# xiph/daala

Measured on AMD Instinct MI355X. Metric: 1080p all-intra transform blocks/s (filter+DCT+PVQ), higher is better.
Workload: dtype int32 (lifting DCT/filters) + f64 (PVQ search)

## Files before the change

### daala_amd/api.py

```python
import ctypes
import os

import numpy as np

_HERE = os.path.dirname(os.path.abspath(__file__))
_LIB = None


class DaalaHipError(RuntimeError):
    pass


EXPERIMENTS_LIB = os.path.join(_HERE, "lib", "libdaalahip_exp.so")


def lib_path():
    return os.environ.get("ODHIP_LIB") or os.path.join(_HERE, "lib", "libdaalahip.so")


def lib():
    global _LIB
    if _LIB is None:
        path = lib_path()
        if not os.path.exists(path):
# ... 515 lines not shown
REFBAND_R_NULL, REFBAND_THETA, REFBAND_NOREF, REFBAND_FLIP, REFBAND_UNCERTAIN = 1, 2, 4, 8, 16
REFITEM_SEARCHED, REFITEM_WITH_REF, REFITEM_K_RANGE = 1, 2, 4
REFITEM_MOMENT_SHIFT = 8


class _RefJob(ctypes.Structure):
    _fields_ = [("d_coef", ctypes.c_void_p), ("d_ref", ctypes.c_void_p), ("nplanes", ctypes.c_int),
                ("w", ctypes.c_int), ("h", ctypes.c_int), ("bs", ctypes.c_int),
                ("is_keyframe", ctypes.c_int), ("pli", ctypes.c_int), ("d_qm", ctypes.c_void_p),
                ("d_qm_inv", ctypes.c_void_p), ("q_band", ctypes.POINTER(ctypes.c_int32)),
                ("beta_band", ctypes.POINTER(ctypes.c_int32)), ("band", ctypes.c_void_p),
                ("items", ctypes.c_void_p), ("y", ctypes.c_void_p), ("r16", ctypes.c_void_p),
                ("x16", ctypes.c_void_p), ("xr", ctypes.c_void_p), ("d_rate", ctypes.c_void_p),
                ("choice", ctypes.c_void_p), ("d_dq", ctypes.c_void_p),
                ("q_band2", ctypes.POINTER(ctypes.c_int32)), ("plane_split", ctypes.c_int),
                ("luma", ctypes.c_void_p), ("d_q_plane", ctypes.c_void_p)]


class PvqRefJob:

    def __init__(self, coef, ref, bs, qm, qm_inv, q_band, beta_band, is_keyframe, pli, rate=None,
                 share=None, q_band2=None, plane_split=0):
        import torch
        _need(coef, torch.int32, "coef")
        _need(ref, torch.int32, "ref")
        assert coef.shape == ref.shape
        self.coef, self.ref, self.bs, self.qm, self.qm_inv = coef, ref, int(bs), qm, qm_inv
        self.is_keyframe, self.pli, self.rate = int(is_keyframe), int(pli), rate
        nplanes, h, w = coef.shape
        n = 4 << bs
        self.nblocks = B = nplanes * (h // n) * (w // n)
# ... 292 lines not shown


PIPE_STAGES = ("image_copy_pad_luma", "forward_pyramid_luma", "pvq_noref_bands", "pvq_choose",
               "cfl_refs_from_luma", "dequant_inverse_luma", "image_copy_pad_chroma",
               "forward_pyramid_chroma", "pvq_ref_bands", "pvq_ref_choose", "dequant_inverse_chroma")
(BUF_PIC, BUF_PX, BUF_LEVEL, BUF_RECON, BUF_BAND, BUF_Y, BUF_CHOICE, BUF_ITEMS, BUF_REF,
 BUF_RATE) = range(10)
BUF_PRED = 10


class _PipeConfig(ctypes.Structure):
    _fields_ = [("device", ctypes.c_int), ("frames", ctypes.c_int), ("pic_w", ctypes.c_int),
                ("pic_h", ctypes.c_int), ("chroma_cfl", ctypes.c_int), ("serial", ctypes.c_int),
                ("price", ctypes.c_int), ("fpr_bits", ctypes.c_int), ("inter", ctypes.c_int),
                ("chroma_444", ctypes.c_int),
                ("pvq_norm_lambda", ctypes.c_double), ("quant", ctypes.c_void_p)]


def export_layout_make(nblocks, bs, with_ref):
    lay = _ExportLayout()
    n = len(bs)
    _check(lib().odhip_export_layout_make(ctypes.byref(lay), n, (ctypes.c_long * n)(*nblocks), (ctypes.c_int * n)(*bs),
                                          (ctypes.c_int * n)(*[int(bool(w)) for w in with_ref])),
           "odhip_export_layout_make")
    return lay, _layout_dict(lay)


def _layout_dict(lay):
    secs = [{k: int(getattr(lay.section[i], k)) for k in ("bs", "ngroups", "cap_words", "blocks_per_group", "record_bytes",
                                                         "nrecords", "records_off", "group_base_off", "stream_off")}
            for i in range(lay.nsections)]
# ... 55 lines not shown
class _ExportSection(ctypes.Structure):
    _fields_ = [("bs", ctypes.c_int32), ("ngroups", ctypes.c_uint32), ("cap_words", ctypes.c_uint32),
                ("blocks_per_group", ctypes.c_uint32), ("record_bytes", ctypes.c_uint32), ("pad", ctypes.c_uint32),
                ("nrecords", ctypes.c_uint64), ("records_off", ctypes.c_uint64),
                ("group_base_off", ctypes.c_uint64), ("stream_off", ctypes.c_uint64)]


class _ExportLayout(ctypes.Structure):
    _fields_ = [("nsections", ctypes.c_int32), ("pad", ctypes.c_int32), ("fixed_bytes", ctypes.c_uint64),
                ("total_bytes", ctypes.c_uint64), ("section", _ExportSection * 16)]


class Pipe:

    def __init__(self, quant, frames, pic_w, pic_h, chroma_cfl=True, serial=False, device=0,
                 pvq_norm_lambda=0.147, price=False, fpr_bits=0, inter=False, chroma_444=False):
        L = lib()
        L.odhip_pipe_create.restype = ctypes.c_void_p
        L.odhip_pipe_theta_reruns.restype = ctypes.c_long
        L.odhip_pipe_price_reruns.restype = ctypes.c_long
        cfg = _PipeConfig(int(device), int(frames), int(pic_w), int(pic_h), int(bool(chroma_cfl)),
                          int(bool(serial)), int(bool(price)), int(fpr_bits), int(bool(inter)),
                          int(bool(chroma_444)),
                          float(pvq_norm_lambda),
                          ctypes.cast(ctypes.byref(quant.c), ctypes.c_void_p))
        self.h = L.odhip_pipe_create(ctypes.byref(cfg))
        if not self.h:
            raise DaalaHipError("odhip_pipe_create failed")
        self.frames, self.pic_w, self.pic_h = int(frames), int(pic_w), int(pic_h)
        self.W, self.H = (pic_w + 63) & ~63, (pic_h + 63) & ~63
        self.chroma_cfl = bool(chroma_cfl)
        self.fpr_bits = int(fpr_bits)
        self.inter = bool(inter)
        self.chroma_444 = bool(chroma_444)
        cdec = 0 if chroma_444 else 1
        self.cw, self.ch = (self.pic_w + cdec) >> cdec, (self.pic_h + cdec) >> cdec
        self.chroma_levels = int(L.odhip_pipe_chroma_levels(self._p()))
        global _pipes
        if _pipes is None:
            import weakref
# ... 561 lines not shown
```

### daala_amd/csrc/lapped_kernels.hip

```cpp
#include "../../include/daala_hip.h"
#include <stdio.h>
#include <stdlib.h>
#include <string.h>
#include <type_traits>
#include "od_ctx.cuh"
#include "od_tile.cuh"
#include "od_pvq_math.cuh"
#include "gen/od_scan_tables.h"

namespace {

__device__ __forceinline__ void od_lds_barrier() {
  asm volatile("s_waitcnt lgkmcnt(0)\n\ts_barrier" ::: "memory");
}

typedef int od_v4i __attribute__((ext_vector_type(4)));
__device__ __forceinline__ void od_store_coef4(od_coeff *p, int4 v) {
#ifdef OD_PYR_STORE_NT
  od_v4i w = {v.x, v.y, v.z, v.w};
  __builtin_nontemporal_store(w, reinterpret_cast<od_v4i *>(p));
#else
  *reinterpret_cast<int4 *>(p) = v;
#endif
}
// ... 595 lines not shown
  int pic_w;
  int pic_h;
  int leaf_bs;
  const int16_t *y;
  const int4 *choice;
  const int16_t *qm_inv;
  long nblocks;
  int len;
  int nb_bands;
  const int16_t *r16;
  const od_coeff *ref;
  int px16;
  int inter;
  int dbg;
  int wide;
};

constexpr int kMaxInvLevels = 5;
struct InverseArgsMulti {
  InverseArgs a[kMaxInvLevels];
  int nplanes;
};

__device__ __attribute__((aligned(16))) unsigned short gInvScanXY[OD_SCAN_LEN];
__device__ unsigned char gInvBandOf[OD_SCAN_LEN];

__device__ __forceinline__ unsigned char od_to_px(int c) {
  return (unsigned char)min(max(((c + 8) >> 4) + 128, 0), 255);
}
__device__ __forceinline__ short od_to_px16(int c) {
  return (short)min(max(c + 2048, 0), 4095);
}
__device__ __forceinline__ void od_store_px(uint8_t *plane, long at, int c, bool px16) {
  if (px16) reinterpret_cast<short *>(plane)[at] = od_to_px16(c);
  else plane[at] = od_to_px(c);
}

struct OdQ16 {
  int sh;
  int sl;
  __device__ __forceinline__ explicit OdQ16(int scale) : sh(scale >> 16), sl(scale & 0xffff) {}
  __device__ __forceinline__ int mul(int y) const { return __mul24(y, sh) + (__mul24(y, sl) >> 16); }
};
__device__ __forceinline__ int od_pulse16(unsigned w, int odd) {
  return odd ? (int)w >> 16 : (int)(w << 16) >> 16;
}

template <int LEAF>
__device__ __forceinline__ int walk_band_of(int j, int &off) {
  int b = 0;
  off = 1;
  if constexpr (LEAF >= 1) {
    if (j >= 16) { b = 1; off = 16; }
    if (j >= 24) { b = 2; off = 24; }
    if (j >= 32) { b = 3; off = 32; }
  }
  if constexpr (LEAF >= 2) {
    if (j >= 64) { b = 4; off = 64; }
    if (j >= 96) { b = 5; off = 96; }
    if (j >= 128) { b = 6; off = 128; }
// ... 391 lines not shown
        const int4 ch = chs[hf];
        const int rnd = (1 << ch.w) >> 1;
        const OdQ16 sc(ch.z);
#pragma unroll
        for (int e = 0; e < 4; e++) {
#pragma unroll
          for (int u = 0; u < 2; u++) {
            const int yv = od_pulse16((unsigned)yd[e], u);
            const int qmi = u ? qd[e] >> 16 : (int)(short)qd[e];
            const int xy = u ? (unsigned)sd[e] >> 16 : sd[e] & 0xffff;
            int v = (__mul24(sc.mul(yv), qmi) + rnd) >> ch.w;
            if (hf == 0 && e == 0 && u == 0 && j0 == 0) v = dc;
            t[base + (xy >> 8)*P + (xy & 255)] = v;
          }
        }
      }
    }
  }
  else {
    load_plane_tile<TILE>(t, a.coef + plane_off, a.w, x0, y0, tid);
  }
  __syncthreads();
  switch (a.leaf_bs) {
    case 0: if constexpr (MINLEAF <= 0 && MAXLEAF >= 0) inverse_leaf<TILE, 0>(t, tid); break;
    case 1: if constexpr (MINLEAF <= 1 && MAXLEAF >= 1) inverse_leaf<TILE, 1>(t, tid); break;
    case 2: if constexpr (MINLEAF <= 2 && MAXLEAF >= 2) inverse_leaf<TILE, 2>(t, tid); break;
    case 3: if constexpr (MINLEAF <= 3 && MAXLEAF >= 3) inverse_leaf<TILE, 3>(t, tid); break;
    default:
      if constexpr (TILE == 64 && MAXLEAF >= 4) inverse_leaf<TILE, 4>(t, tid);
      break;
// ... 73 lines not shown
#pragma unroll
      for (int e = 0; e < 4; e++) {
#pragma unroll
        for (int u = 0; u < 2; u++) {
          const int yv = od_pulse16((unsigned)yd[e], u);
          const int qmi = u ? qd[e] >> 16 : (int)(short)qd[e];
          const int xy = u ? (unsigned)sd[e] >> 16 : sd[e] & 0xffff;
          int v = (__mul24(sc.mul(yv), qmi) + rnd) >> ch.w;
          if (hf == 0 && e == 0 && u == 0 && j0 == 0) v = dc;
          tt[base + (xy >> 8)*P + (xy & 255)] = v;
        }
      }
    }
  }
  __syncthreads();
  if (a.leaf_bs == 3) {
    const int s2 = tid >> 7;
    const int lt = tid & 127;
    od_tile_rows<TILE, 3, true, T, 128>(t[s2], t[s2], lt, OdAllBlocks());
    __syncthreads();
    od_tile_cols<TILE, 3, true, T, 128>(t[s2], t[s2], lt, OdAllBlocks());
    __syncthreads();
  }
  else {
    const int g = tid >> 6;
    if (tid < 64) {
      int *tt = t[tid >> 5];
      const int base = (tid & 31)*P;
      T in[64];
      T out[64];
// ... 730 lines not shown
    if constexpr (SRC == 1) {
      if (!OD_INV_DBG(a, 4)) {
        if (!ahead) {
          f.heads(a, plane, plane_off, xg, y0, tid);
          f.pulses(a, plane, xg, y0, tid);
        }
        if constexpr (Fetch::len < Fetch::n*Fetch::n) {
          walk_zero<TILE, G, NT>(t, tid);
          od_lds_barrier();
        }
        if (leaf4) f.commit_leaf4(t, a, tid);
        else f.commit(t, a, tid);
      }
      else walk_zero<TILE, G, NT>(t, tid);
      od_lds_barrier();
      if (ahead && g + 1 < g1) f.heads(a, plane, plane_off, xg + G*TILE, y0, tid);
    }
    else if (leaf4) {
      if constexpr (LEAF == 0 && SRC == 2) walk_leaf4<TILE, G, NT, SRC>(t, a, plane, plane_off, xg, y0, tid);
      od_lds_barrier();
    }
    else {
      if (OD_INV_DBG(a, 4)) walk_zero<TILE, G, NT>(t, tid);
      else if constexpr (SRC == 0) walk_load_plane<TILE, G, NT>(t, a.coef + plane_off, a.w, xg, y0, tid);
      else if constexpr (SRC == 2) walk_load_ref<TILE, G, NT, LEAF>(t, a, plane, plane_off, xg, y0, tid);
      od_lds_barrier();
    }
    if (!leaf4 && !OD_INV_DBG(a, 16)) {
      walk_idct_pass<TILE, G, NT, LEAF, true>(t, tid);
      od_lds_barrier();
// ... 553 lines not shown
  return inverse_launch(ia, nlevels, nplanes, dec, (hipStream_t)stream);
}

extern "C" int odhip_inverse_level_pvq(uint8_t *d_px, int px_stride, long px_plane_stride,
 const odhip_pvq_job *job, int dec, int pic_w, int pic_h, odhip_stream stream) {
  InverseArgs ia;
  int rc = pvq_inverse_args(ia, d_px, px_stride, px_plane_stride, job, dec, pic_w, pic_h);
  if (rc) return rc;
  rc = upload_inv_tables();
  if (rc) return rc;
  return inverse_launch(ia, job->nplanes, dec, (hipStream_t)stream);
}

extern "C" int odhip_inverse_levels_pvq(uint8_t *const *d_px, int px_stride, long px_plane_stride,
 const odhip_pvq_job *jobs, int njobs, int dec, int pic_w, int pic_h, odhip_stream stream) {
  if (!d_px || !jobs || njobs <= 0 || njobs > kMaxInvLevels) return ODHIP_EINVAL;
  InverseArgs ia[kMaxInvLevels];
  for (int i = 0; i < njobs; i++) {
    const int rc = pvq_inverse_args(ia[i], d_px[i], px_stride, px_plane_stride, &jobs[i], dec, pic_w,
     pic_h);
    if (rc) return rc;
    if (jobs[i].nplanes != jobs[0].nplanes || jobs[i].w != jobs[0].w || jobs[i].h != jobs[0].h) {
      return ODHIP_EINVAL;
    }
  }
  const int rc = upload_inv_tables();
  if (rc) return rc;
  return inverse_launch(ia, njobs, jobs[0].nplanes, dec, (hipStream_t)stream);
}

extern "C" int odhip_inverse_levels_pvq_ref(uint8_t *const *d_px, int px_stride, long px_plane_stride,
 const odhip_pvq_refjob *jobs, int njobs, int dec, int pic_w, int pic_h, odhip_stream stream) {
  if (!d_px || !jobs || njobs <= 0 || njobs > kMaxInvLevels || (dec != 0 && dec != 1)) return ODHIP_EINVAL;
  InverseArgs ia[kMaxInvLevels];
  for (int i = 0; i < njobs; i++) {
    const odhip_pvq_refjob &j = jobs[i];
    const bool lref = j.luma != nullptr && j.is_keyframe && j.pli != 0;
    if ((!j.d_ref && !lref) || !j.r16 || ((uintptr_t)j.r16 & 15) || j.nplanes != jobs[0].nplanes || j.w != jobs[0].w
// ... 16 lines not shown
```

### daala_amd/csrc/pipeline.hip

```cpp
#include <stdio.h>
#include <stdlib.h>
#include <string.h>
#include <atomic>
#include <chrono>
#include <vector>
#include "od_ctx.cuh"
#include "gen/od_scan_tables.h"

namespace {

constexpr int kStages = ODHIP_PIPE_NSTAGES;
constexpr int kMaxTimed = 4096;

struct PlaneSet {
  int dec;
  int pli;
  int nplanes;
  int w, h;
  int pw, ph;
  int nlev;
  uint8_t *pic;
  uint8_t *pic_buf[2];
  uint8_t *px;
  uint8_t *pred_pic;
// ... 52 lines not shown

struct odhip_pipe {
  odhip_pipe_config cfg = {};
  int pic_w = 0, pic_h = 0, W = 0, H = 0;
  odhip_ctx *ctx[2] = {};
  hipStream_t stream[2] = {};
  bool serial = false;
  PlaneSet set[2] = {};
  int cdec = 1;
  odhip_pvq_job jobs[2][2*ODHIP_NBSIZES] = {};
  int njobs = 0;
  odhip_pvq_refjob refjobs[2][ODHIP_NBSIZES] = {};
  odhip_pvq_refjob interjobs[2][ODHIP_NBSIZES] = {};
  bool inter_pending[2] = {};
  double *rate[2][ODHIP_NBSIZES] = {};
  hipEvent_t ev_refs[2] = {};
  hipEvent_t ev_used[2] = {};
  long nstep = 0;
  int pending = -1;
  long reruns = 0;
  long price_reruns = 0;
  double wait_ms = 0;
  long k_range = 0;
  bool record = false;
  hipStream_t copy_stream = nullptr;
  hipEvent_t ev_fed = nullptr;
  hipEvent_t ev_pad[2] = {};
  int front = 0;
  bool fed = false;
  hipStream_t export_stream = nullptr;
// ... 225 lines not shown
  }
  p->njobs = 0;
  return ODHIP_SUCCESS;
}

int setup_keyframe_jobs(odhip_pipe *p) {
  PlaneSet &ch = p->set[1];
  for (int bs = 0; bs < 5; bs++) STEP_TRY(setup_job(p, p->jobs[0][bs], p->set[0], bs));
  p->njobs = 5;
  if (!p->cfg.chroma_cfl) {
    for (int bs = 0; bs < ch.nlev; bs++) STEP_TRY(setup_job(p, p->jobs[0][5 + bs], ch, bs));
    p->njobs = 5 + ch.nlev;
    return ODHIP_SUCCESS;
  }
  for (int bs = 0; bs < 5; bs++) STEP_TRY(setup_job(p, p->jobs[1][bs], p->set[0], bs, &p->jobs[0][bs]));
  for (int par = 0; par < 2; par++) {
    for (int bs = 0; bs < ch.nlev; bs++) {
      STEP_TRY(setup_refjob(p, p->refjobs[par][bs], ch, bs, nullptr, par ? &p->refjobs[0][bs] : nullptr,
       &p->jobs[par][bs + ch.dec]));
    }
    STEP_TRY(pipe_event(p, &p->ev_refs[par]));
    STEP_TRY(pipe_event(p, &p->ev_used[par]));
  }
  return ODHIP_SUCCESS;
}

int pipe_init(odhip_pipe *p) {
  const odhip_pipe_config &c = p->cfg;
  ODHIP_TRY(hipSetDevice(c.device));
  p->pic_w = c.pic_w;
  p->pic_h = c.pic_h;
  p->W = (c.pic_w + 63) & ~63;
  p->H = (c.pic_h + 63) & ~63;
  p->serial = c.serial || odhip_env_serial();
// ... 190 lines not shown
}

int stage_pad_run(odhip_pipe *p, int si, hipStream_t s) {
  Timed tm(p, si ? ODHIP_PIPE_PAD_CHROMA : ODHIP_PIPE_PAD_LUMA, s);
  return pad_planes(p, si, p->set[si].px, p->set[si].pic, s);
}

int stage_pyramid(odhip_pipe *p, int si, hipStream_t s) {
  Timed tm(p, si ? ODHIP_PIPE_PYRAMID_CHROMA : ODHIP_PIPE_PYRAMID_LUMA, s);
  return pyramid(p, si, p->set[si].levels, p->set[si].px, s);
}

int stage_inverse_noref(odhip_pipe *p, int si, hipStream_t s, int jpar) {
  PlaneSet &t = p->set[si];
  Timed tm(p, si ? ODHIP_PIPE_INVERSE_CHROMA : ODHIP_PIPE_INVERSE_LUMA, s);
  return odhip_inverse_levels_pvq(t.recon, t.w, (long)t.w*t.h, p->jobs[jpar] + (si ? 5 : 0), t.nlev, t.dec,
   p->pic_w, p->pic_h, s);
}

int ref_bands(odhip_pipe *p, int si, int par, hipStream_t s) {
  const double lam = p->cfg.pvq_norm_lambda;
  const int nlev = p->set[si].nlev;
  Timed tm(p, si ? ODHIP_PIPE_BANDS_CHROMA : ODHIP_PIPE_BANDS_LUMA, s);
  if (p->cfg.price) return odhip_pvq_ref_bands_decided_multi(ref_jobs(p, si, par), nlev, lam, s);
  STEP_TRY(odhip_pvq_ref_bands_multi(ref_jobs(p, si, par), nlev, lam, s));
  return odhip_pvq_ref_resolve_begin(s);
}

int ref_choose(odhip_pipe *p, int si, int par, hipStream_t s) {
  Timed tm(p, si ? ODHIP_PIPE_CHOOSE_CHROMA : ODHIP_PIPE_CHOOSE_LUMA, s);
  return odhip_pvq_ref_choose_multi(ref_jobs(p, si, par), p->set[si].nlev, p->cfg.pvq_norm_lambda, s);
}

int ref_inverse(odhip_pipe *p, int si, int par, hipStream_t s) {
  const PlaneSet &t = p->set[si];
  Timed tm(p, si ? ODHIP_PIPE_INVERSE_CHROMA : ODHIP_PIPE_INVERSE_LUMA, s);
  return odhip_inverse_levels_pvq_ref(t.recon, t.w, (long)t.w*t.h, ref_jobs(p, si, par), t.nlev, t.dec, p->pic_w,
   p->pic_h, s);
}

// ... 297 lines not shown
  }
  return ODHIP_SUCCESS;
}

int step_cfl(odhip_pipe *p) {
  hipStream_t main = p->stream[0];
  hipStream_t side = p->stream[1];
  const int par = (int)(p->nstep & 1);
  const bool exp_on = exporting(p);
  quants_point(p, 0, par);
  {
    Current cur(p->ctx[0]);
    STEP_TRY(luma_front(p, main, par));
    STEP_TRY(luma_choose(p, main, par));
    if (exp_on) ODHIP_TRY(hipStreamWaitEvent(main, p->ev_exp_sent[par], 0));
    ODHIP_TRY(hipEventRecord(p->ev_refs[par], main));
    if (exp_on) STEP_TRY(export_luma(p, par));
    STEP_TRY(stage_inverse_noref(p, 0, main, par));
    STEP_TRY(measure(p, 0, par, main));
  }
  STEP_TRY(finish_pending(p));
  if (exp_on) STEP_TRY(export_finish(p));
  STEP_TRY(metrics_finish(p, side));
  {
    Current cur(p->ctx[1]);
    STEP_TRY(stage_pad(p, 1, side));
    STEP_TRY(stage_pyramid(p, 1, side));
    ODHIP_TRY(hipStreamWaitEvent(side, p->ev_refs[par], 0));
    quants_point(p, 1, par);
    STEP_TRY(quants_upload(p, 1, par, side));
    STEP_TRY(ref_bands(p, 1, par, side));
    ODHIP_TRY(hipEventRecord(p->ev_used[par], side));
    if (exp_on) STEP_TRY(export_chroma(p, par));
    STEP_TRY(ref_tail(p, 1, par, side));
  }
  p->pending = par;
  metrics_step_done(p, par);
  return ODHIP_SUCCESS;
}

}

extern "C" odhip_pipe *odhip_pipe_create(const odhip_pipe_config *cfg) {
  if (!cfg || !cfg->quant || cfg->frames <= 0 || cfg->pic_w <= 0 || cfg->pic_h <= 0
   || (cfg->chroma_444 != 0 && cfg->chroma_444 != 1)
   || (!cfg->chroma_444 && ((cfg->pic_w & 1) || (cfg->pic_h & 1)))
// ... 519 lines not shown
    case ODHIP_PIPE_BUF_Y:
      ptr = j ? j->cands.y : r->y;
      n = sizeof(int16_t)*(size_t)(j ? 2 : ODHIP_PVQ_REF_SLOTS)*B*len;
      break;
    case ODHIP_PIPE_BUF_CHOICE:
      ptr = j ? j->cands.choice : r->choice;
      n = sizeof(int32_t)*(size_t)B*nb*(j ? 4 : 16);
      break;
    case ODHIP_PIPE_BUF_ITEMS:
      if (!r) return ODHIP_EINVAL;
      ptr = r->items;
      n = (size_t)3*nb*ODHIP_PVQ_REF_SLOTS*B*16;
      break;
    case ODHIP_PIPE_BUF_REF:
      if (!r) return ODHIP_EINVAL;
      if (!inter) return ODHIP_EINVAL;
      ptr = t.pred_levels[level];
      n = sizeof(od_coeff)*(size_t)t.nplanes*t.w*t.h;
      break;
    case ODHIP_PIPE_BUF_RATE: {
      n = sizeof(double)*(size_t)B*nb*(j ? 2 : ODHIP_PVQ_REF_SLOTS + 1);
      if (!p->rate[set][level]) {
        ODHIP_TRY(hipSetDevice(p->cfg.device));
        PIPE_ALLOC(p, p->rate[set][level], n, true);
        for (int par = 0; par < 2; par++) {
          const JobAt a = job_at(p, set, level, par);
          if (a.ref) a.ref->d_rate = p->rate[set][level];
          else a.noref->d_rate = p->rate[set][level];
        }
      }
      ptr = p->rate[set][level];
// ... 238 lines not shown
```

### daala_amd/csrc/pvq_refbands.hip

```cpp
#include "../../include/daala_hip.h"
#include <math.h>
#include <stdio.h>
#include <stdlib.h>
#include <string.h>
#include "od_ctx.cuh"
#include "od_pvq_math.cuh"
#include "od_occupancy.cuh"
#include "od_krange.cuh"
#include "od_band_stage.cuh"
#include "gen/od_scan_tables.h"
#define OD_RSQ_TABLE_N 512
#define OD_RSQ_HUGE
#include "pvq_search.cuh"
#include "pvq_row.cuh"
#include "pvq_regs.cuh"

namespace {

constexpr int kMaxJobs = 8;
constexpr int kMaxItems = kMaxJobs*ODHIP_MAX_BANDS;
constexpr int kSlots = ODHIP_PVQ_REF_SLOTS;
constexpr int kUncCap = 1 << 16;
constexpr double kDefaultMargin = 1e-9;

// ... 27 lines not shown
  int pli;
  int q[ODHIP_MAX_BANDS];
  int beta[ODHIP_MAX_BANDS];
  int off[ODHIP_MAX_BANDS + 1];
  long split_blk;
  int q2[ODHIP_MAX_BANDS];
  const int *qp;
  unsigned plane_blocks;
  const int16_t *ly;
  const int32_t *lchoice;
  const int16_t *lqmi;
  long lnblocks;
  long lsplit;
  int llen;
  int lnb;
};

__device__ __forceinline__ int job_q(const RJob &jb, int band, long blk) {
  const int q = blk >= jb.split_blk ? jb.q2[band] : jb.q[band];
  return q ? q : jb.qp[(unsigned)blk/jb.plane_blocks*ODHIP_MAX_BANDS + band];
}

__device__ __forceinline__ void lref_piece(const RJob &jb, int band, long blk, int c0, int (&rv)[8]) {
  const long lblk = blk >= jb.lsplit ? blk - jb.lsplit : blk;
  const int4 ch = reinterpret_cast<const int4 *>(jb.lchoice)[lblk*jb.lnb + band];
  uint4 y4 = make_uint4(0, 0, 0, 0);
  if (ch.y != 0) y4 = *reinterpret_cast<const uint4 *>(jb.ly + ((long)ch.x*jb.lnblocks + lblk)*jb.llen + c0);
  const uint4 q4 = *reinterpret_cast<const uint4 *>(jb.lqmi + c0);
  const unsigned yw[4] = {y4.x, y4.y, y4.z, y4.w};
  const unsigned qw[4] = {q4.x, q4.y, q4.z, q4.w};
#pragma unroll
// ... 240 lines not shown
  const RJob &jb = it.jobs[job];
  const int band = it.band[item];
  const long blk = (long)(blockIdx.x - it.wg_start[item])*kWave + threadIdx.x;
  if (blk >= jb.nblocks) return;
  const int off = jb.off[band];
  const int w = jb.w;
  const int len = jb.len;
  const int nb_bands = jb.nb_bands;
  const int q0 = job_q(jb, band, blk);
  const int beta = jb.beta[band];
  const int is_keyframe = jb.is_keyframe;
  const int cfl_enabled = is_keyframe && jb.pli != 0;
  const long base = block_base(jb, blk);
  const od_coeff *x0 = jb.coef + base;
  const bool lref = jb.ly != nullptr;
  const od_coeff *r0 = lref ? jb.coef + base : jb.ref + base;
  const int16_t *qmp = jb.qm + off;
  odhip_pvq_refband *rec = jb.rec + blk*nb_bands;
  int16_t *x16o = jb.x16 + blk*len;
  int16_t *r16o = jb.r16 + blk*len;
  int16_t *xro = jb.xr + blk*len;
  int xv[N];
  int rv[N];
  int qm[N];
  if constexpr (N == 15) {
    int4 xr4[4];
    int4 rr4[4];
#pragma unroll
    for (int y = 0; y < 4; y++) {
      xr4[y] = *reinterpret_cast<const int4 *>(x0 + (long)y*w);
      rr4[y] = lref ? make_int4(0, 0, 0, 0) : *reinterpret_cast<const int4 *>(r0 + (long)y*w);
// ... 216 lines not shown
  const int l = lane%G;
  const long nblocks = jb.nblocks;
  const long blk0 = (long)(blockIdx.x - it.wg_start[item])*(kWave/G) + row;
  const bool live = blk0 < nblocks;
  const long blk = live ? blk0 : nblocks - 1;
  const int w = jb.w;
  const int len = jb.len;
  const int nb_bands = jb.nb_bands;
  const int q0 = job_q(jb, band, blk);
  const int beta = jb.beta[band];
  const int is_keyframe = jb.is_keyframe;
  const int cfl_enabled = is_keyframe && jb.pli != 0;
  const long base = block_base(jb, blk);
  const od_coeff *x0 = jb.coef + base;
  const bool lref = jb.ly != nullptr;
  const od_coeff *r0 = lref ? jb.coef + base : jb.ref + base;
  const int16_t *qmp = jb.qm + off + l*E;
  odhip_pvq_refband *rec = jb.rec + blk*nb_bands;
  int16_t *x16o = jb.x16 + blk*len + off;
  int16_t *r16o = jb.r16 + blk*len + off;
  int16_t *xro = jb.xr + blk*len + off;
  const int flip = cfl_enabled ? (rec[0].flags & ODHIP_REFBAND_FLIP) != 0 : 0;
  int xv[E];
  int rv[E];
  int qm[E];
  int sx = 0;
  int sr = 0;
  int nz = 0;
#pragma unroll
  for (int e = 0; e < E; e++) {
    const int pk = s_scan[l*E + e];
// ... 1653 lines not shown
    return ODHIP_EINVAL;
  }
  if (((uintptr_t)j.band & 63) || ((uintptr_t)j.items & 15) || ((uintptr_t)j.y & 15)
   || ((uintptr_t)j.r16 & 15) || ((uintptr_t)j.x16 & 15) || ((uintptr_t)j.xr & 15)
   || ((uintptr_t)j.choice & 15)) {
    return ODHIP_EINVAL;
  }
  if (mode == 0 ? (!j.d_qm || !j.x16 || !j.xr) : mode == 1 ? (!j.d_qm_inv || !j.choice || !j.d_dq)
   : !j.choice) {
    return ODHIP_EINVAL;
  }
  const int n = 4 << j.bs;
  if (j.w <= 0 || j.h <= 0 || j.w % n || j.h % n) return ODHIP_EINVAL;
  if (mode == 0 && (((uintptr_t)j.d_coef & 15) || ((uintptr_t)j.d_ref & 15))) return ODHIP_EINVAL;
  if (j.luma && !j.d_ref && mode == 1) return ODHIP_EINVAL;
  memset(&d, 0, sizeof(d));
  d.coef = j.d_coef;
  d.ref = j.d_ref;
  d.qm = j.d_qm;
  d.qm_inv = j.d_qm_inv;
  d.rec = j.band;
  d.items = j.items;
  d.y = j.y;
  d.r16 = j.r16;
  d.x16 = j.x16;
  d.xr = j.xr;
  d.rate = j.d_rate;
  d.choice = j.choice;
  d.dq = j.d_dq;
  d.nplanes = j.nplanes;
// ... 12 lines not shown
  for (int i = 0; i < d.nb_bands; i++) {
    if (j.q_band[i] < 1) return ODHIP_EINVAL;
    d.q[i] = j.q_band[i];
    d.q2[i] = j.q_band[i];
    d.beta[i] = j.beta_band[i];
  }
  d.split_blk = d.nblocks;
  if (j.q_band2) {
    if (j.plane_split <= 0 || j.plane_split >= j.nplanes) return ODHIP_EINVAL;
    d.split_blk = (long)j.plane_split*d.bw*d.bh;
    for (int i = 0; i < d.nb_bands; i++) {
      if (j.q_band2[i] < 1) return ODHIP_EINVAL;
      d.q2[i] = j.q_band2[i];
    }
  }
  d.qp = j.d_q_plane;
  d.plane_blocks = (unsigned)(d.bw*d.bh);
  if (d.qp) {
    for (int i = 0; i < d.nb_bands; i++) d.q[i] = d.q2[i] = 0;
  }
  if (j.luma) {
    const odhip_pvq_job &l = *j.luma;
    const bool up = l.bs == j.bs + 1 && l.w == 2*j.w && l.h == 2*j.h;
    const bool same = l.bs == j.bs && l.w == j.w && l.h == j.h;
    if ((!up && !same) || !l.cands.y || !l.cands.choice || !l.d_qm_inv
     || (l.nplanes != j.nplanes && 2*l.nplanes != j.nplanes) || !j.is_keyframe || j.pli == 0
     || ((uintptr_t)l.cands.y & 15) || ((uintptr_t)l.cands.choice & 15) || ((uintptr_t)l.d_qm_inv & 15)) {
      return ODHIP_EINVAL;
    }
    const int ln = 4 << l.bs;
// ... 568 lines not shown
```

### include/daala_hip.h

```cpp
#ifndef DAALA_HIP_H
#define DAALA_HIP_H
#include <stddef.h>
#include <stdint.h>

#ifdef __cplusplus
extern "C" {
#endif

typedef int32_t od_coeff;

#define ODHIP_SUCCESS (0)
#define ODHIP_EFAULT (-1)
#define ODHIP_EINVAL (-10)
#define ODHIP_EIMPL (-23)
#define ODHIP_ERANGE (-24)
#define ODHIP_EBUSY (-101)

#define ODHIP_NBSIZES 5

typedef void *odhip_stream;


typedef void (*odhip_dct_func_2d)(od_coeff *out, int out_stride,
 const od_coeff *in, int in_stride);
// ... 158 lines not shown
 double pvq_norm_lambda, odhip_stream stream);

int odhip_inverse_level_pvq(uint8_t *d_px, int px_stride, long px_plane_stride,
 const odhip_pvq_job *job, int dec, int pic_w, int pic_h, odhip_stream stream);

int odhip_cfl_refs_from_luma(const odhip_pvq_job *luma_jobs, int njobs, od_coeff *const *d_ref,
 int copies, odhip_stream stream);
int odhip_cfl_refs_from_luma_ex(const odhip_pvq_job *luma_jobs, int njobs, od_coeff *const *d_ref,
 int copies, int prezeroed, odhip_stream stream);

int odhip_pvq_profile(int enable);
int odhip_pvq_profile_read(float *ms, int max_n);

int odhip_inverse_levels_pvq(uint8_t *const *d_px, int px_stride, long px_plane_stride,
 const odhip_pvq_job *jobs, int njobs, int dec, int pic_w, int pic_h, odhip_stream stream);

int odhip_pvq_band_layout(int bs, int *nb_bands, int *offsets, int *len);

int odhip_pvq_noref_bands(const od_coeff *d_coef, int nplanes, int w, int h,
 int bs, const int16_t *d_qm, const int32_t *q_band, const int32_t *beta_band,
 double pvq_norm_lambda, const odhip_pvq_cands *out, odhip_stream stream);

int odhip_pvq_select_synth_noref(od_coeff *d_dq, const od_coeff *d_coef,
 int nplanes, int w, int h, int bs, const int16_t *d_qm_inv,
 const int32_t *q_band, const int32_t *beta_band, double pvq_norm_lambda,
 const odhip_pvq_cands *in, const double *d_rate, int32_t *d_qg_out,
 odhip_stream stream);

typedef struct {
  int32_t xshift, rshift;
// ... 76 lines not shown
  const int32_t *q_band;
  const int32_t *beta_band;
  odhip_pvq_refband *band;
  void *items;
  int16_t *y;
  int16_t *r16;
  int16_t *x16;
  int16_t *xr;
  const double *d_rate;
  int32_t *choice;
  od_coeff *d_dq;
  const int32_t *q_band2;
  int plane_split;
  const struct odhip_pvq_job_s *luma;
  const int32_t *d_q_plane;
} odhip_pvq_refjob;

int odhip_pvq_ref_set_context(int ctx);
int odhip_pvq_ref_bands_multi(const odhip_pvq_refjob *jobs, int njobs,
 double pvq_norm_lambda, odhip_stream stream);
int odhip_pvq_ref_resolve(const odhip_pvq_refjob *jobs, int njobs,
 double pvq_norm_lambda, odhip_stream stream);
int odhip_pvq_ref_resolve_begin(odhip_stream stream);
int odhip_pvq_ref_resolve_finish(const odhip_pvq_refjob *jobs, int njobs,
 double pvq_norm_lambda, odhip_stream stream);
int odhip_pvq_ref_select_synth_multi(const odhip_pvq_refjob *jobs, int njobs,
 double pvq_norm_lambda, odhip_stream stream);
int odhip_pvq_ref_profile(int enable);
int odhip_pvq_ref_profile_read(float *ms, int max_n);
int odhip_pvq_ref_choose_multi(const odhip_pvq_refjob *jobs, int njobs,
// ... 120 lines not shown

typedef struct odhip_pipe odhip_pipe;
typedef struct {
  int device;
  int frames;
  int pic_w;
  int pic_h;
  int chroma_cfl;
  int serial;
  int price;
  int fpr_bits;
  int inter;
  int chroma_444;
  double pvq_norm_lambda;
  const odhip_quant *quant;
} odhip_pipe_config;
enum {
  ODHIP_PIPE_PAD_LUMA = 0, ODHIP_PIPE_PYRAMID_LUMA, ODHIP_PIPE_BANDS_LUMA, ODHIP_PIPE_CHOOSE_LUMA,
  ODHIP_PIPE_CFL_REFS, ODHIP_PIPE_INVERSE_LUMA, ODHIP_PIPE_PAD_CHROMA, ODHIP_PIPE_PYRAMID_CHROMA,
  ODHIP_PIPE_BANDS_CHROMA, ODHIP_PIPE_CHOOSE_CHROMA, ODHIP_PIPE_INVERSE_CHROMA, ODHIP_PIPE_NSTAGES
};
enum {
  ODHIP_PIPE_BUF_PIC = 0,
  ODHIP_PIPE_BUF_PX,
  ODHIP_PIPE_BUF_LEVEL,
  ODHIP_PIPE_BUF_RECON,
  ODHIP_PIPE_BUF_BAND,
  ODHIP_PIPE_BUF_Y,
  ODHIP_PIPE_BUF_CHOICE,
  ODHIP_PIPE_BUF_ITEMS,
// ... 171 lines not shown
```

Baseline: 1.161 billion.

## Emit CfL chroma reference planes from luma inverse and share across Cb/Cr

During the luma inverse pass the kernel now writes decimated CfL reference coefficient planes straight from LDS tiles into per-level buffers. Chroma ref-band search then reads these planes directly, and Cb and Cr share one reference via a block-index offset, replacing the per-block gather from luma jobs. The chroma side stream now waits until after the luma inverse instead of after luma choose, which delays chroma start and may cost overlap. It also adds extra global stores and barriers to the inverse kernel.

New measurement: 1.125 billion. -3.1%, worse.

```diff
diff --git a/daala_amd/api.py b/daala_amd/api.py
--- a/daala_amd/api.py
+++ b/daala_amd/api.py
@@ -553,7 +553,8 @@
                 ("x16", ctypes.c_void_p), ("xr", ctypes.c_void_p), ("d_rate", ctypes.c_void_p),
                 ("choice", ctypes.c_void_p), ("d_dq", ctypes.c_void_p),
                 ("q_band2", ctypes.POINTER(ctypes.c_int32)), ("plane_split", ctypes.c_int),
-                ("luma", ctypes.c_void_p), ("d_q_plane", ctypes.c_void_p)]
+                ("luma", ctypes.c_void_p), ("d_q_plane", ctypes.c_void_p),
+                ("ref_planes", ctypes.c_int)]
 
 
 class PvqRefJob:
@@ -876,7 +877,8 @@
                 ("pic_h", ctypes.c_int), ("chroma_cfl", ctypes.c_int), ("serial", ctypes.c_int),
                 ("price", ctypes.c_int), ("fpr_bits", ctypes.c_int), ("inter", ctypes.c_int),
                 ("chroma_444", ctypes.c_int),
-                ("pvq_norm_lambda", ctypes.c_double), ("quant", ctypes.c_void_p)]
+                ("pvq_norm_lambda", ctypes.c_double), ("quant", ctypes.c_void_p),
+                ("cfl_gather", ctypes.c_int)]
 
 
 def export_layout_make(nblocks, bs, with_ref):
@@ -962,7 +964,8 @@
 class Pipe:
 
     def __init__(self, quant, frames, pic_w, pic_h, chroma_cfl=True, serial=False, device=0,
-                 pvq_norm_lambda=0.147, price=False, fpr_bits=0, inter=False, chroma_444=False):
+                 pvq_norm_lambda=0.147, price=False, fpr_bits=0, inter=False, chroma_444=False,
+                 cfl_gather=False):
         L = lib()
         L.odhip_pipe_create.restype = ctypes.c_void_p
         L.odhip_pipe_theta_reruns.restype = ctypes.c_long
@@ -971,7 +974,7 @@
                           int(bool(serial)), int(bool(price)), int(fpr_bits), int(bool(inter)),
                           int(bool(chroma_444)),
                           float(pvq_norm_lambda),
-                          ctypes.cast(ctypes.byref(quant.c), ctypes.c_void_p))
+                          ctypes.cast(ctypes.byref(quant.c), ctypes.c_void_p), int(bool(cfl_gather)))
         self.h = L.odhip_pipe_create(ctypes.byref(cfg))
         if not self.h:
             raise DaalaHipError("odhip_pipe_create failed")
diff --git a/daala_amd/csrc/lapped_kernels.hip b/daala_amd/csrc/lapped_kernels.hip
--- a/daala_amd/csrc/lapped_kernels.hip
+++ b/daala_amd/csrc/lapped_kernels.hip
@@ -633,6 +633,7 @@
   int inter;
   int dbg;
   int wide;
+  od_coeff *cfl;
 };
 
 constexpr int kMaxInvLevels = 5;
@@ -663,6 +664,28 @@
 };
 __device__ __forceinline__ int od_pulse16(unsigned w, int odd) {
   return odd ? (int)w >> 16 : (int)(w << 16) >> 16;
+}
+
+template <int G, int NT, int P>
+__device__ __forceinline__ void cfl_store(const int *t, int tile_words, const InverseArgs &a, int leaf, int plane,
+ int x0, int y0, unsigned tid) {
+  constexpr int TILE = 64;
+  constexpr int Q = G*TILE/8;
+  const int nsh = leaf + 1;
+  const unsigned nm = (1u << nsh) - 1;
+  const int cw = a.w >> 1;
+  od_coeff *out = a.cfl + ((long)plane*(a.h >> 1) + (y0 >> 1))*cw + (x0 >> 1);
+  for (unsigned i = tid; i < (unsigned)(TILE/2*Q); i += NT) {
+    const unsigned cy = i/Q;
+    const unsigned cx = (i % Q)*4;
+    const unsigned s = cx/(TILE/2);
+    const unsigned cxl = cx % (TILE/2);
+    const unsigned ly = ((cy >> nsh) << (nsh + 1)) | (cy & nm);
+    const unsigned lx = ((cxl >> nsh) << (nsh + 1)) | (cxl & nm);
+    int4 v = *reinterpret_cast<const int4 *>(t + s*tile_words + ly*P + lx);
+    if (!(cy & nm) && !(cxl & nm)) v.x = 0;
+    *reinterpret_cast<int4 *>(out + (long)cy*cw + cx) = v;
+  }
 }
 
 template <int LEAF>
@@ -1084,6 +1107,12 @@
             t[base + (xy >> 8)*P + (xy & 255)] = v;
           }
         }
+      }
+    }
+    if constexpr (TILE == 64) {
+      if (a.cfl) {
+        od_lds_barrier();
+        cfl_store<1, NT, P>(t, 0, a, a.leaf_bs, plane, x0, y0, tid);
       }
     }
   }
@@ -1187,6 +1216,10 @@
     }
   }
   __syncthreads();
+  if (a.cfl) {
+    cfl_store<2, NT, P>(&t[0][0], TILE*P, a, a.leaf_bs, plane, xb, y0, tid);
+    od_lds_barrier();
+  }
   if (a.leaf_bs == 3) {
     const int s2 = tid >> 7;
     const int lt = tid & 127;
@@ -1947,6 +1980,12 @@
       }
       else walk_zero<TILE, G, NT>(t, tid);
       od_lds_barrier();
+      if constexpr (TILE == 64 && G == 1 && LEAF >= 1) {
+        if (a.cfl) {
+          cfl_store<G, NT, P>(t, TILE*P, a, LEAF, plane, xg, y0, tid);
+          od_lds_barrier();
+        }
+      }
       if (ahead && g + 1 < g1) f.heads(a, plane, plane_off, xg + G*TILE, y0, tid);
     }
     else if (leaf4) {
@@ -2530,7 +2569,12 @@
 
 extern "C" int odhip_inverse_levels_pvq(uint8_t *const *d_px, int px_stride, long px_plane_stride,
  const odhip_pvq_job *jobs, int njobs, int dec, int pic_w, int pic_h, odhip_stream stream) {
-  if (!d_px || !jobs || njobs <= 0 || njobs > kMaxInvLevels) return ODHIP_EINVAL;
+  return odhip_inverse_levels_pvq_cfl(d_px, px_stride, px_plane_stride, jobs, njobs, dec, pic_w, pic_h, nullptr, stream);
+}
+
+extern "C" int odhip_inverse_levels_pvq_cfl(uint8_t *const *d_px, int px_stride, long px_plane_stride,
+ const odhip_pvq_job *jobs, int njobs, int dec, int pic_w, int pic_h, od_coeff *const *d_cfl, odhip_stream stream) {
+  if (!d_px || !jobs || njobs <= 0 || njobs > kMaxInvLevels || (d_cfl && dec)) return ODHIP_EINVAL;
   InverseArgs ia[kMaxInvLevels];
   for (int i = 0; i < njobs; i++) {
     const int rc = pvq_inverse_args(ia[i], d_px[i], px_stride, px_plane_stride, &jobs[i], dec, pic_w,
@@ -2538,6 +2582,10 @@
     if (rc) return rc;
     if (jobs[i].nplanes != jobs[0].nplanes || jobs[i].w != jobs[0].w || jobs[i].h != jobs[0].h) {
       return ODHIP_EINVAL;
+    }
+    if (d_cfl && d_cfl[i] && jobs[i].bs >= 1) {
+      if ((uintptr_t)d_cfl[i] & 15) return ODHIP_EINVAL;
+      ia[i].cfl = d_cfl[i];
     }
   }
   const int rc = upload_inv_tables();
diff --git a/daala_amd/csrc/pipeline.hip b/daala_amd/csrc/pipeline.hip
--- a/daala_amd/csrc/pipeline.hip
+++ b/daala_amd/csrc/pipeline.hip
@@ -90,6 +90,8 @@
   odhip_pvq_refjob interjobs[2][ODHIP_NBSIZES] = {};
   bool inter_pending[2] = {};
   double *rate[2][ODHIP_NBSIZES] = {};
+  od_coeff *cfl_plane[2][ODHIP_NBSIZES] = {};
+  bool cfl_planes = false;
   hipEvent_t ev_refs[2] = {};
   hipEvent_t ev_used[2] = {};
   long nstep = 0;
@@ -345,10 +347,15 @@
     return ODHIP_SUCCESS;
   }
   for (int bs = 0; bs < 5; bs++) STEP_TRY(setup_job(p, p->jobs[1][bs], p->set[0], bs, &p->jobs[0][bs]));
+  const char *gather = ODHIP_EXP_ENV("ODHIP_CFL_GATHER");
+  p->cfl_planes = ch.dec == 1 && !p->cfg.cfl_gather && !(gather && atoi(gather) != 0);
   for (int par = 0; par < 2; par++) {
     for (int bs = 0; bs < ch.nlev; bs++) {
       STEP_TRY(setup_refjob(p, p->refjobs[par][bs], ch, bs, nullptr, par ? &p->refjobs[0][bs] : nullptr,
        &p->jobs[par][bs + ch.dec]));
+      if (p->cfl_planes) {
+        PIPE_ALLOC(p, p->cfl_plane[par][bs], sizeof(od_coeff)*(size_t)p->set[0].nplanes*ch.w*ch.h, true);
+      }
     }
     STEP_TRY(pipe_event(p, &p->ev_refs[par]));
     STEP_TRY(pipe_event(p, &p->ev_used[par]));
@@ -569,16 +576,31 @@
 int stage_inverse_noref(odhip_pipe *p, int si, hipStream_t s, int jpar) {
   PlaneSet &t = p->set[si];
   Timed tm(p, si ? ODHIP_PIPE_INVERSE_CHROMA : ODHIP_PIPE_INVERSE_LUMA, s);
-  return odhip_inverse_levels_pvq(t.recon, t.w, (long)t.w*t.h, p->jobs[jpar] + (si ? 5 : 0), t.nlev, t.dec,
-   p->pic_w, p->pic_h, s);
-}
-
-int ref_bands(odhip_pipe *p, int si, int par, hipStream_t s) {
+  od_coeff *cfl[ODHIP_NBSIZES] = {};
+  if (si == 0 && p->cfl_planes) {
+    for (int bs = 1; bs < t.nlev; bs++) cfl[bs] = p->cfl_plane[jpar][bs - 1];
+  }
+  return odhip_inverse_levels_pvq_cfl(t.recon, t.w, (long)t.w*t.h, p->jobs[jpar] + (si ? 5 : 0), t.nlev, t.dec,
+   p->pic_w, p->pic_h, si == 0 && p->cfl_planes ? cfl : nullptr, s);
+}
+
+int ref_bands(odhip_pipe *p, int si, int par, hipStream_t s, bool planes = false) {
   const double lam = p->cfg.pvq_norm_lambda;
   const int nlev = p->set[si].nlev;
   Timed tm(p, si ? ODHIP_PIPE_BANDS_CHROMA : ODHIP_PIPE_BANDS_LUMA, s);
-  if (p->cfg.price) return odhip_pvq_ref_bands_decided_multi(ref_jobs(p, si, par), nlev, lam, s);
-  STEP_TRY(odhip_pvq_ref_bands_multi(ref_jobs(p, si, par), nlev, lam, s));
+  const odhip_pvq_refjob *jobs = ref_jobs(p, si, par);
+  odhip_pvq_refjob pj[ODHIP_NBSIZES];
+  if (planes) {
+    for (int bs = 0; bs < nlev; bs++) {
+      pj[bs] = jobs[bs];
+      pj[bs].luma = nullptr;
+      pj[bs].d_ref = p->cfl_plane[par][bs];
+      pj[bs].ref_planes = p->set[0].nplanes;
+    }
+    jobs = pj;
+  }
+  if (p->cfg.price) return odhip_pvq_ref_bands_decided_multi(jobs, nlev, lam, s);
+  STEP_TRY(odhip_pvq_ref_bands_multi(jobs, nlev, lam, s));
   return odhip_pvq_ref_resolve_begin(s);
 }
 
@@ -906,9 +928,10 @@
     STEP_TRY(luma_front(p, main, par));
     STEP_TRY(luma_choose(p, main, par));
     if (exp_on) ODHIP_TRY(hipStreamWaitEvent(main, p->ev_exp_sent[par], 0));
-    ODHIP_TRY(hipEventRecord(p->ev_refs[par], main));
+    if (!p->cfl_planes) ODHIP_TRY(hipEventRecord(p->ev_refs[par], main));
     if (exp_on) STEP_TRY(export_luma(p, par));
     STEP_TRY(stage_inverse_noref(p, 0, main, par));
+    if (p->cfl_planes) ODHIP_TRY(hipEventRecord(p->ev_refs[par], main));
     STEP_TRY(measure(p, 0, par, main));
   }
   STEP_TRY(finish_pending(p));
@@ -921,7 +944,7 @@
     ODHIP_TRY(hipStreamWaitEvent(side, p->ev_refs[par], 0));
     quants_point(p, 1, par);
     STEP_TRY(quants_upload(p, 1, par, side));
-    STEP_TRY(ref_bands(p, 1, par, side));
+    STEP_TRY(ref_bands(p, 1, par, side, p->cfl_planes));
     ODHIP_TRY(hipEventRecord(p->ev_used[par], side));
     if (exp_on) STEP_TRY(export_chroma(p, par));
     STEP_TRY(ref_tail(p, 1, par, side));
@@ -1471,7 +1494,12 @@
       break;
     case ODHIP_PIPE_BUF_REF:
       if (!r) return ODHIP_EINVAL;
-      if (!inter) return ODHIP_EINVAL;
+      if (!inter) {
+        if (set != 1 || !p->cfl_planes) return ODHIP_EINVAL;
+        ptr = p->cfl_plane[parity][level];
+        n = sizeof(od_coeff)*(size_t)p->set[0].nplanes*t.w*t.h;
+        break;
+      }
       ptr = t.pred_levels[level];
       n = sizeof(od_coeff)*(size_t)t.nplanes*t.w*t.h;
       break;
diff --git a/daala_amd/csrc/pvq_refbands.hip b/daala_amd/csrc/pvq_refbands.hip
--- a/daala_amd/csrc/pvq_refbands.hip
+++ b/daala_amd/csrc/pvq_refbands.hip
@@ -65,7 +65,13 @@
   long lsplit;
   int llen;
   int lnb;
+  long rsplit;
+  long rback;
 };
+
+__device__ __forceinline__ long ref_base(const RJob &jb, long blk, long base) {
+  return blk >= jb.rsplit ? base - jb.rback : base;
+}
 
 __device__ __forceinline__ int job_q(const RJob &jb, int band, long blk) {
   const int q = blk >= jb.split_blk ? jb.q2[band] : jb.q[band];
@@ -336,7 +342,7 @@
   const long base = block_base(jb, blk);
   const od_coeff *x0 = jb.coef + base;
   const bool lref = jb.ly != nullptr;
-  const od_coeff *r0 = lref ? jb.coef + base : jb.ref + base;
+  const od_coeff *r0 = lref ? jb.coef + base : jb.ref + ref_base(jb, blk, base);
   const int16_t *qmp = jb.qm + off;
   odhip_pvq_refband *rec = jb.rec + blk*nb_bands;
   int16_t *x16o = jb.x16 + blk*len;
@@ -583,7 +589,7 @@
   const long base = block_base(jb, blk);
   const od_coeff *x0 = jb.coef + base;
   const bool lref = jb.ly != nullptr;
-  const od_coeff *r0 = lref ? jb.coef + base : jb.ref + base;
+  const od_coeff *r0 = lref ? jb.coef + base : jb.ref + ref_base(jb, blk, base);
   const int16_t *qmp = jb.qm + off + l*E;
   odhip_pvq_refband *rec = jb.rec + blk*nb_bands;
   int16_t *x16o = jb.x16 + blk*len + off;
@@ -2267,6 +2273,8 @@
   if (j.w <= 0 || j.h <= 0 || j.w % n || j.h % n) return ODHIP_EINVAL;
   if (mode == 0 && (((uintptr_t)j.d_coef & 15) || ((uintptr_t)j.d_ref & 15))) return ODHIP_EINVAL;
   if (j.luma && !j.d_ref && mode == 1) return ODHIP_EINVAL;
+  const bool rshare = j.ref_planes != 0 && j.ref_planes != j.nplanes;
+  if (rshare && (2*j.ref_planes != j.nplanes || !j.d_ref || !j.is_keyframe || j.pli == 0 || mode == 1)) return ODHIP_EINVAL;
   memset(&d, 0, sizeof(d));
   d.coef = j.d_coef;
   d.ref = j.d_ref;
@@ -2309,6 +2317,8 @@
       d.q2[i] = j.q_band2[i];
     }
   }
+  d.rsplit = rshare ? (long)j.ref_planes*d.bw*d.bh : d.nblocks;
+  d.rback = rshare ? (long)j.ref_planes*j.w*j.h : 0;
   d.qp = j.d_q_plane;
   d.plane_blocks = (unsigned)(d.bw*d.bh);
   if (d.qp) {
diff --git a/include/daala_hip.h b/include/daala_hip.h
--- a/include/daala_hip.h
+++ b/include/daala_hip.h
@@ -196,6 +196,9 @@
 
 int odhip_inverse_levels_pvq(uint8_t *const *d_px, int px_stride, long px_plane_stride,
  const odhip_pvq_job *jobs, int njobs, int dec, int pic_w, int pic_h, odhip_stream stream);
+int odhip_inverse_levels_pvq_cfl(uint8_t *const *d_px, int px_stride, long px_plane_stride,
+ const odhip_pvq_job *jobs, int njobs, int dec, int pic_w, int pic_h, od_coeff *const *d_cfl,
+ odhip_stream stream);
 
 int odhip_pvq_band_layout(int bs, int *nb_bands, int *offsets, int *len);
 
@@ -302,6 +305,7 @@
   int plane_split;
   const struct odhip_pvq_job_s *luma;
   const int32_t *d_q_plane;
+  int ref_planes;
 } odhip_pvq_refjob;
 
 int odhip_pvq_ref_set_context(int ctx);
@@ -452,6 +456,7 @@
   int chroma_444;
   double pvq_norm_lambda;
   const odhip_quant *quant;
+  int cfl_gather;
 } odhip_pipe_config;
 enum {
   ODHIP_PIPE_PAD_LUMA = 0, ODHIP_PIPE_PYRAMID_LUMA, ODHIP_PIPE_BANDS_LUMA, ODHIP_PIPE_CHOOSE_LUMA,
```
